# ggirelli/kman

Hardware: NVIDIA B200
Metric: k-mers/sec (extract+sort+count, k=31) (higher is better)
Workload: dtype u64

## Files before the change

### kman_b200/csrc/common.cuh

```cuda
#pragma once
#include <cuda_runtime.h>
#include <stdint.h>
#include <stdio.h>
#include <string.h>

#include <type_traits>

#include "../../include/kmg.h"

namespace kmg {

void set_error(const char* fmt, ...);
void bump_launches(int n = 1);

#define KMG_CUDA(call)                                                                          \
    do {                                                                                        \
        cudaError_t e__ = (call);                                                               \
        if (e__ != cudaSuccess) {                                                               \
            kmg::set_error("%s:%d: %s -> %s", __FILE__, __LINE__, #call, cudaGetErrorString(e__)); \
            return KMG_ERR_CUDA;                                                                \
        }                                                                                       \
    } while (0)

#define KMG_REQUIRE(cond, code, ...)    \
// ... 29 lines not shown
static inline PassPlan make_plan(int begin_bit, int end_bit) {
    PassPlan plan;
    memset(&plan, 0, sizeof(plan));
    const int bits = end_bit - begin_bit;
    const int np = (bits + SORT_RADIX_BITS - 1) / SORT_RADIX_BITS;
    plan.num_passes = np;
    for (int i = 0; i < np; ++i) {
        plan.shift[i] = begin_bit + i * SORT_RADIX_BITS;
        plan.bits[i] = i + 1 < np ? SORT_RADIX_BITS : bits - i * SORT_RADIX_BITS;
    }
    return plan;
}

struct CountOut {
    uint32_t* counts;
    unsigned long long* n_out;
    bool done;
};
struct PrePartitioned {
    int pb;
    const unsigned long long* top;
    const unsigned long long* bucket_starts = nullptr;
    bool in_alt = false;
};
size_t top_hist_workspace_bytes();
int extract_top_hist(const uint8_t* d_bases, uint64_t n_bases, uint64_t win_begin, uint64_t win_end, int k, int rc,
                     const uint8_t* d_lut256, uint64_t* d_counts, unsigned long long* d_top, unsigned long long* d_plan,
                     void* d_ws, size_t ws_bytes, cudaStream_t st);
constexpr size_t P16_ZEROED_WORDS = 65536 + 3 * 256 + 4;
static inline unsigned long long* p16_top(unsigned long long* zeroed) { return zeroed + 65536; }
static inline unsigned long long* p16_plan(unsigned long long* zeroed) { return zeroed + 65536 + 3 * 256; }
struct Prefix16Out {
    unsigned long long* zeroed;
    unsigned long long* region_starts;
    unsigned long long* starts;
    unsigned long long* cursors;
    uint32_t* rows;
};
size_t prefix16_rows_bytes();
int extract_prefix16_hist(const uint8_t* d_bases, uint64_t n_bases, uint64_t win_begin, uint64_t win_end, int k, int rc,
                          const uint8_t* d_lut256, const Prefix16Out& o, cudaStream_t st);
int region_partition(const void* d_keys_in, void* d_keys_out, const void* d_vals_in, void* d_vals_out, uint64_t n,
                     int key_bytes, int val_bytes, const unsigned long long* d_region_counts, unsigned long long* d_cursors,
                     int digit_shift, cudaStream_t st);
int extract_digit_scatter(const uint8_t* d_bases, uint64_t n_bases, uint64_t win_begin, uint64_t win_end, int k, int rc,
                          const uint8_t* d_lut256, void* d_keys_out, int key_bytes, void* d_vals_out, int val_bytes,
                          uint64_t pos_offset, unsigned long long* d_cursors, int digit_shift, cudaStream_t st);
bool hybrid_sort_applies(uint64_t n, int key_bytes, int val_bytes, int end_bit, bool pairs_ok);
int hybrid_choose_pb(uint64_t n, unsigned long long max_top_byte_count, int key_bytes, int val_bytes);
int sort_count_core(void* d_keys, void* d_keys_alt, uint64_t n, int key_bytes, int end_bit, const uint64_t* d_hist_in,
                    uint32_t* d_counts_out, uint64_t* d_n_out, int* h_selector_out, void* d_ws, size_t ws_bytes, void* stream,
                    const PrePartitioned* pre);
int sort_uniq_core(void* d_keys, void* d_keys_alt, void* d_vals, void* d_vals_alt, uint64_t n, int key_bytes, int val_bytes,
                   int end_bit, const uint64_t* d_hist_in, uint64_t* d_n_out, int* h_selector_out, void* d_ws,
                   size_t ws_bytes, void* stream, const PrePartitioned* pre);
void exclusive_scan_256(const unsigned long long* d_hist_row, unsigned long long* d_out, cudaStream_t st);
extern thread_local int64_t g_stat_last_n_out, g_stat_last_err;
void timing_begin(cudaStream_t st);
void timing_end(cudaStream_t st, int kind);

struct __align__(16) u128 {
    uint64_t lo, hi;
};

__host__ __device__ __forceinline__ bool operator==(const u128& a, const u128& b) { return a.lo == b.lo && a.hi == b.hi; }
__host__ __device__ __forceinline__ bool operator!=(const u128& a, const u128& b) { return !(a == b); }
__host__ __device__ __forceinline__ bool operator<(const u128& a, const u128& b) {
    return a.hi < b.hi || (a.hi == b.hi && a.lo < b.lo);
}

struct __align__(16) u256 {
    u128 lo, hi;
// ... 152 lines not shown
__device__ __forceinline__ void mbar_expect_tx(uint64_t* bar, uint32_t bytes) {
    asm volatile("mbarrier.arrive.expect_tx.shared::cta.b64 _, [%0], %1;" ::"r"(smem_u32(bar)), "r"(bytes) : "memory");
}
__device__ __forceinline__ void mbar_wait(uint64_t* bar, uint32_t parity) {
    asm volatile(
        "{\n"
        ".reg .pred p;\n"
        "WAIT_LOOP:\n"
        "mbarrier.try_wait.parity.shared::cta.b64 p, [%0], %1;\n"
        "@p bra WAIT_DONE;\n"
        "bra WAIT_LOOP;\n"
        "WAIT_DONE:\n"
        "}\n" ::"r"(smem_u32(bar)),
        "r"(parity)
        : "memory");
}
__device__ __forceinline__ void tma_load_1d(void* smem_dst, const void* gmem_src, uint32_t bytes, uint64_t* bar) {
    asm volatile("cp.async.bulk.shared::cluster.global.mbarrier::complete_tx::bytes [%0], [%1], %2, [%3];" ::"r"(
                     smem_u32(smem_dst)),
                 "l"(gmem_src), "r"(bytes), "r"(smem_u32(bar))
                 : "memory");
}

__device__ __forceinline__ void tma_prefetch_l2(const void* gmem_src, uint32_t bytes) {
    asm volatile("cp.async.bulk.prefetch.L2.global [%0], %1;" ::"l"(gmem_src), "r"(bytes) : "memory");
}

__device__ __forceinline__ uint32_t lane_id() { return threadIdx.x & 31; }
__device__ __forceinline__ uint32_t lanemask_lt() {
    uint32_t m;
    asm("mov.u32 %0, %%lanemask_lt;" : "=r"(m));
    return m;
}

template <typename T>
__device__ __forceinline__ T warp_incl_scan(T v) {
#pragma unroll
    for (int o = 1; o < 32; o <<= 1) {
        T t = __shfl_up_sync(0xffffffffu, v, o);
        if (lane_id() >= (uint32_t)o) v += t;
    }
    return v;
}

template <int BLOCK, typename T>
__device__ __forceinline__ T block_excl_scan(T v, T* smem, T& total) {
// ... 18 lines not shown
```

### kman_b200/csrc/extract.cu

```cuda
#include "extract_tile.cuh"

namespace kmg {

constexpr int EX_BLOCK_DEFAULT = 256;

struct ExtractParams {
    const uint8_t* bases;
    uint64_t n_bases;
    uint64_t win_begin, win_end;
    uint64_t first_tile;
    int k;
    const uint8_t* lut;
    const uint8_t* comp16;
    void* keys_out;
    void* vals_out;
    uint64_t pos_offset;
    unsigned long long* counts;
    uint64_t* tile_state;
    uint32_t* ticket;
    uint32_t* err;
    unsigned long long* hs;
    int n_off;
    int hist_off[2 * MAX_PASSES];
    unsigned long long* cursors;
// ... 13 lines not shown
__device__ __forceinline__ uint32_t mer4_at(uint64_t X0, uint64_t X1, uint64_t X2, int e) {
    const int w = e >> 5, off = 2 * (e & 31);
    const uint64_t a = w == 0 ? X0 : (w == 1 ? X1 : X2);
    const uint64_t b = w == 0 ? X1 : (w == 1 ? X2 : 0ull);
    const uint64_t v = off == 0 ? a : ((a << off) | (b >> (64 - off)));
    return (uint32_t)(v >> 56);
}
__device__ __forceinline__ bool plain4_at(uint64_t B0, uint64_t B1, int e) {
    uint64_t v;
    if (e == 0) v = B0;
    else if (e < 64) v = (B0 << e) | (B1 >> (64 - e));
    else v = B1 << (e - 64);
    return (v >> 60) == 0;
}

template <int BLOCK>
struct DigitRuns {
    uint32_t* s_cnt;
    uint32_t* s_off;
    unsigned long long* s_gb;
    uint32_t* s_scan;

    __device__ __forceinline__ uint32_t rank(uint32_t d) const { return d | (atomicAdd(&s_cnt[d], 1u) << 8); }
    __device__ __forceinline__ uint32_t reserve(unsigned long long* cursors) const {
        const int t = threadIdx.x;
        const uint32_t c = t < 256 ? s_cnt[t] : 0u;
        unsigned long long g = 0;
        if (c) g = atomicAdd(&cursors[t], (unsigned long long)c);
        uint32_t n_tile;
        const uint32_t off = block_excl_scan<BLOCK, uint32_t>(c, s_scan, n_tile);
        if (t < 256) {
            s_off[t] = off;
            s_gb[t] = g - off;
        }
        __syncthreads();
        return n_tile;
    }
    __device__ __forceinline__ uint32_t slot(uint32_t wh) const { return s_off[wh & 255u] + (wh >> 8); }
    template <bool PAY, typename KeyT, typename ValT, typename DigitOf>
    __device__ __forceinline__ void write_runs(const KeyT* s_keys, const ValT* s_vals, uint32_t n_tile, DigitOf digit_of,
                                               KeyT* keys_out, ValT* vals_out) const {
        for (uint32_t i = threadIdx.x; i < n_tile; i += BLOCK) {
            const KeyT key = s_keys[i];
            const unsigned long long at = s_gb[digit_of(key)] + i;
            keys_out[at] = key;
            if constexpr (PAY) vals_out[at] = s_vals[i];
        }
    }
};

template <typename KeyT, int PPT, bool RC, int VAL_BYTES, bool HIST, int MODE, int EX_BLOCK, bool FILTER = false>
// ... 112 lines not shown
        }
    }
    if constexpr (MODE == 1) {
        __syncthreads();
        if (t == 0) {
            if (total) atomicAdd(&p.counts[0], (unsigned long long)total * OUT_PER_WIN);
            if (s_wide) atomicAdd(&p.counts[1], (unsigned long long)s_wide);
        }
        return;
    }

    if constexpr (MODE == 2) {
        const int dsh = p.digit_shift;
        const DigitRuns<EX_BLOCK> runs{s_cnt, s_off, s_gb, s_scan};
        uint32_t wh[PPT * OUT_PER_WIN];
#pragma unroll
        for (int j = 0; j < PPT; ++j) {
            if (!(vf & (1u << j))) continue;
            const KeyT key = build_key<KeyT>(X0, X1, X2, joff + j, k);
            wh[j * OUT_PER_WIN] = runs.rank(key_digit(key, dsh, 255u));
            if constexpr (RC) wh[j * 2 + 1] = runs.rank(key_digit(rc_key(key, k), dsh, 255u));
        }
        __syncthreads();
        const uint32_t n_tile = runs.reserve(p.cursors);
#pragma unroll
        for (int j = 0; j < PPT; ++j) {
            if (!(vf & (1u << j))) continue;
            const KeyT key = build_key<KeyT>(X0, X1, X2, joff + j, k);
            const uint64_t pos = tile_pos + (uint64_t)t * PPT + j + p.pos_offset;
            const uint32_t i0 = runs.slot(wh[j * OUT_PER_WIN]);
            s_keys[i0] = key;
            if constexpr (VAL_BYTES != 0) s_vals[i0] = make_val<ValT>(pos, 0);
            if constexpr (RC) {
                const uint32_t i1 = runs.slot(wh[j * 2 + 1]);
                s_keys[i1] = rc_key(key, k);
                if constexpr (VAL_BYTES != 0) s_vals[i1] = make_val<ValT>(pos, 1);
            }
        }
        __syncthreads();
        runs.template write_runs<VAL_BYTES != 0>(s_keys, s_vals, n_tile, [dsh](const KeyT& key) { return key_digit(key, dsh, 255u); },
                                                 reinterpret_cast<KeyT*>(p.keys_out), reinterpret_cast<ValT*>(p.vals_out));
        return;
    }

    uint32_t r = excl;
#pragma unroll
    for (int j = 0; j < PPT; ++j) {
// ... 407 lines not shown
    if (t < 256) {
        s_lut[t] = p.lut[t];
        s_b3[t] = 0;
    }
    if (t < 2) s_n[t] = 0;
    const int k = p.k;
    uint32_t n_valid = 0, n_wide = 0;
    for (uint32_t tile = blockIdx.x; tile < p.n_tiles; tile += gridDim.x) {
        __syncthreads();
        const uint64_t tile_pos = (p.first_tile + tile) * P16_TILE;
        encode_tile_words<P16_BLOCK, WORDS>(p.bases, p.n_bases, t, tile_pos, s_lut, s_codes, s_bad, s_inv);
        __syncthreads();
        const auto [X0, X1, X2, B0, B1, I0, I1] = load_tile_words(s_codes, s_bad, s_inv, t);
        uint32_t in_range_mask, nwide;
        bool span_clean;
        const uint32_t vf = narrow_window_flags<P16_PPT>(tile_pos + (uint64_t)t * P16_PPT, p.win_begin, p.win_end, k, 0, B0, B1,
                                                         I0, I1, in_range_mask, span_clean, nwide);
        n_valid += __popc(vf);
        n_wide += nwide;
#pragma unroll
        for (int j = 0; j < P16_PPT; ++j) {
            if (!(vf & (1u << j))) continue;
            count16(s_h, p.spill, mer8_at(X0, X1, X2, j));
            atomicAdd(&s_b3[mer4_at(X0, X1, X2, j + 8)], 1u);
            if constexpr (RC) {
                count16(s_h, p.spill, rc8(mer8_at(X0, X1, X2, j + k - 8)));
                atomicAdd(&s_b3[rc4(mer4_at(X0, X1, X2, j + k - 12))], 1u);
            }
        }
    }
#pragma unroll
    for (int o = 16; o > 0; o >>= 1) {
        n_valid += __shfl_xor_sync(0xffffffffu, n_valid, o);
        n_wide += __shfl_xor_sync(0xffffffffu, n_wide, o);
    }
    if ((t & 31) == 0) {
        if (n_valid) atomicAdd(&s_n[0], (unsigned long long)n_valid);
        if (n_wide) atomicAdd(&s_n[1], (unsigned long long)n_wide);
    }
    __syncthreads();
    uint4* row = reinterpret_cast<uint4*>(p.rows + (size_t)blockIdx.x * P16_WORDS);
    for (uint32_t i = t; i < P16_WORDS / 4; i += P16_BLOCK) row[i] = reinterpret_cast<const uint4*>(s_h)[i];
    if (t < 256 && s_b3[t]) atomicAdd(&p.byte3[t], (unsigned long long)s_b3[t]);
    if (t < 2 && s_n[t]) atomicAdd(&p.counts[t], s_n[t]);
}

__global__ void __launch_bounds__(256) prefix16_reduce_kernel(const uint32_t* __restrict__ rows, int n_rows,
                                                              const unsigned long long* __restrict__ spill,
                                                              unsigned long long* __restrict__ top,
                                                              unsigned long long* __restrict__ starts) {
    __shared__ unsigned long long s_scan[256 / 32 + 1];
    const uint32_t r = blockIdx.x, t = threadIdx.x, b = r * 256 + t;
    const uint32_t* w = rows + (b >> 1);
    const int sh = (int)(b & 1u) << 4;
    uint32_t acc = 0;
#pragma unroll 8
    for (int c = 0; c < n_rows; ++c) acc += (w[(size_t)c * P16_WORDS] >> sh) & 0xFFFFu;
    const unsigned long long v = spill[b] + acc;
    unsigned long long tot;
    const unsigned long long ex = block_excl_scan<256, unsigned long long>(v, s_scan, tot);
    starts[b] = ex;
    if (t == 0) top[2 * 256 + r] = tot;
    if (v) atomicAdd(&top[256 + t], v);
}

__global__ void __launch_bounds__(256) prefix16_starts_kernel(const unsigned long long* __restrict__ top,
                                                              unsigned long long* __restrict__ plan,
                                                              unsigned long long* __restrict__ region_starts,
                                                              unsigned long long* __restrict__ starts,
                                                              unsigned long long* __restrict__ cursors) {
    __shared__ unsigned long long s_scan[256 / 32 + 1], s_max[8], s_base;
    const uint32_t r = blockIdx.x, t = threadIdx.x, b = r * 256 + t;
    const unsigned long long c = top[2 * 256 + t];
    unsigned long long total;
    const unsigned long long ex = block_excl_scan<256, unsigned long long>(c, s_scan, total);
    if (t == r) s_base = ex;
    __syncthreads();
    const unsigned long long s = starts[b] + s_base;
    starts[b] = s;
    cursors[b] = s;
    if (t == 0) region_starts[r] = s_base;
    if (r == 0) {
        unsigned long long mx = c;
#pragma unroll
        for (int o = 16; o > 0; o >>= 1) mx = max(mx, __shfl_xor_sync(0xffffffffu, mx, o));
        if ((t & 31) == 0) s_max[t >> 5] = mx;
        __syncthreads();
        if (t == 0) {
            for (int i = 1; i < 8; ++i) mx = max(mx, s_max[i]);
            plan[0] = total;
            plan[1] = mx;
            starts[65536] = total;
        }
    }
}

constexpr int RP_BLOCK = 512;
template <typename KeyT, int VB>
constexpr int rp_ipt() { return sizeof(KeyT) == 8 ? (VB == 0 ? 12 : 8) : (VB == 8 ? 6 : 8); }

struct RegionPartParams {
    const void* keys_in;
    void* keys_out;
    const void* vals_in;
    void* vals_out;
    const unsigned long long* counts;
    unsigned long long* cursors;
    int digit_shift;
};

template <typename KeyT, int VB>
__global__ void __launch_bounds__(RP_BLOCK, 2) region_partition_kernel(const RegionPartParams p) {
    constexpr int IPT = rp_ipt<KeyT, VB>();
    constexpr uint32_t TILE = RP_BLOCK * IPT;
    using ValT = typename std::conditional<VB == 4, uint32_t, uint64_t>::type;
    extern __shared__ __align__(16) unsigned char smem_raw[];
    KeyT* s_keys = reinterpret_cast<KeyT*>(smem_raw);
    ValT* s_vals = reinterpret_cast<ValT*>(smem_raw + sizeof(KeyT) * TILE);
    __shared__ uint32_t s_cnt[256], s_off[256];
    __shared__ unsigned long long s_gb[256];
    __shared__ uint32_t s_scan[RP_BLOCK / 32 + 1];
    __shared__ unsigned long long s_scan64[RP_BLOCK / 32 + 1];
    __shared__ uint32_t s_region;
    __shared__ unsigned long long s_lo, s_hi;

    const int t = threadIdx.x;
    const unsigned long long c = t < 256 ? p.counts[t] : 0ull;
    const uint32_t nt = (uint32_t)((c + TILE - 1) / TILE);
    uint32_t tiles_all;
    unsigned long long keys_all;
    const uint32_t t0 = block_excl_scan<RP_BLOCK, uint32_t>(nt, s_scan, tiles_all);
    const unsigned long long k0 = block_excl_scan<RP_BLOCK, unsigned long long>(c, s_scan64, keys_all);
    if (blockIdx.x >= tiles_all) return;
    if (t < 256) s_cnt[t] = 0;
    if (blockIdx.x - t0 < nt) {
        s_region = t;
        s_lo = k0 + (unsigned long long)(blockIdx.x - t0) * TILE;
        s_hi = k0 + c;
    }
    __syncthreads();
    const uint32_t r = s_region;
    const unsigned long long lo = s_lo;
    const uint32_t n_in = (uint32_t)min((unsigned long long)TILE, s_hi - lo);
    const KeyT* keys_in = reinterpret_cast<const KeyT*>(p.keys_in) + lo;
    const ValT* vals_in = reinterpret_cast<const ValT*>(p.vals_in) + lo;
    const int dsh = p.digit_shift;
    const DigitRuns<RP_BLOCK> runs{s_cnt, s_off, s_gb, s_scan};
    KeyT key[IPT];
    ValT val[VB ? IPT : 1];
    uint32_t wh[IPT];
#pragma unroll
    for (int q = 0; q < IPT; ++q) {
        const uint32_t i = q * RP_BLOCK + t;
        if (i < n_in) {
            key[q] = keys_in[i];
            if constexpr (VB != 0) val[q] = vals_in[i];
        }
    }
#pragma unroll
    for (int q = 0; q < IPT; ++q)
        if (q * RP_BLOCK + t < n_in) wh[q] = runs.rank(key_digit(key[q], dsh, 255u));
    __syncthreads();
    const uint32_t n_tile = runs.reserve(p.cursors + (size_t)r * 256);
#pragma unroll
    for (int q = 0; q < IPT; ++q) {
        if (q * RP_BLOCK + t < n_in) {
            const uint32_t i = runs.slot(wh[q]);
            s_keys[i] = key[q];
            if constexpr (VB != 0) s_vals[i] = val[q];
        }
    }
    __syncthreads();
    runs.template write_runs<VB != 0>(s_keys, s_vals, n_tile, [dsh](const KeyT& k_) { return key_digit(k_, dsh, 255u); },
                                      reinterpret_cast<KeyT*>(p.keys_out), reinterpret_cast<ValT*>(p.vals_out));
}

template <typename KeyT, int VB>
static int launch_region_partition(const RegionPartParams& p, uint64_t n, cudaStream_t st) {
    constexpr uint64_t TILE = (uint64_t)RP_BLOCK * rp_ipt<KeyT, VB>();
    const uint64_t grid = (n + TILE - 1) / TILE + 256;
    KMG_REQUIRE(grid < (1ull << 31), KMG_ERR_RANGE, "too many tiles");
    const size_t smem = TILE * (sizeof(KeyT) + VB);
    auto kern = region_partition_kernel<KeyT, VB>;
    KMG_CUDA(cudaFuncSetAttribute(kern, cudaFuncAttributeMaxDynamicSharedMemorySize, (int)smem));
    kern<<<(uint32_t)grid, RP_BLOCK, smem, st>>>(p);
    KMG_LAUNCH_CHECK();
    return KMG_OK;
}

template <bool RC, int LIMBS, int FILTER = 0>
static int dispatch_wide(const ExtractParams& p, uint32_t n_tiles, int vb, cudaStream_t st) {
    if (vb == 0) extract_wide_kernel<RC, 0, LIMBS, FILTER><<<n_tiles, EXW_BLOCK, 0, st>>>(p);
    else if (vb == 4) extract_wide_kernel<RC, 4, LIMBS, FILTER><<<n_tiles, EXW_BLOCK, 0, st>>>(p);
    else extract_wide_kernel<RC, 8, LIMBS, FILTER><<<n_tiles, EXW_BLOCK, 0, st>>>(p);
    KMG_LAUNCH_CHECK();
    return KMG_OK;
}
template <int FILTER>
static int dispatch_wide_any(const ExtractParams& p, uint32_t n_tiles, int k, int rc, int vb, cudaStream_t st) {
    if (k <= 32) return rc ? dispatch_wide<true, 2, FILTER>(p, n_tiles, vb, st) : dispatch_wide<false, 2, FILTER>(p, n_tiles, vb, st);
    return rc ? dispatch_wide<true, 4, FILTER>(p, n_tiles, vb, st) : dispatch_wide<false, 4, FILTER>(p, n_tiles, vb, st);
}

static void fill_common(ExtractParams& p, const uint8_t* d_bases, uint64_t n_bases, uint64_t win_begin, uint64_t win_end,
                        uint64_t tile, int k, const uint8_t* d_lut256) {
// ... 308 lines not shown
```

### kman_b200/csrc/pipeline.cu

```cuda
#include <algorithm>

#include "common.cuh"

extern "C" size_t kmg_rle_workspace_bytes(uint64_t n);

namespace kmg {

namespace {
struct PipeWs {
    unsigned long long* zeroed;
    unsigned long long* top;
    unsigned long long* plan;
    unsigned long long* cursors;
    unsigned long long* starts;
    unsigned long long* cursors16;
    uint32_t* rows;
    uint64_t* hist16;
    uint64_t* n_out;
    void* ex_ws;
    size_t ex_ws_bytes;
    void* sort_ws;
    size_t sort_ws_bytes;
    size_t total;
};
// ... 77 lines not shown
    if (fused) {
        timing_begin(st);
        const Prefix16Out p16{w.zeroed, w.cursors, w.starts, w.cursors16, w.rows};
        rcode = extract_prefix16_hist(d_bases, n_bases, win_begin, win_end, k, rc, d_lut256, p16, st);
        timing_end(st, 2);
        if (rcode != KMG_OK) return rcode;
        unsigned long long h_plan[4] = {0, 0, 0, 0};
        KMG_CUDA(cudaMemcpyAsync(h_plan, w.plan, sizeof(h_plan), cudaMemcpyDeviceToHost, st));
        KMG_CUDA(cudaStreamSynchronize(st));
        n = h_plan[0];
        h_result[1] = n;
        h_result[2] = h_plan[3];
        KMG_REQUIRE(h_plan[2] * (rc ? 2 : 1) == n, KMG_ERR_STATE,
                    "prefix histogram (%llu keys) disagrees with the window count (%llu)", h_plan[0],
                    h_plan[2] * (rc ? 2 : 1));
        if (n == 0) return KMG_OK;
        fused = hybrid_sort_applies(n, kb, val_bytes, 2 * k, true);
        if (fused) {
            PrePartitioned pre;
            pre.pb = hybrid_choose_pb(n, h_plan[1], kb, val_bytes);
            pre.top = w.top;
            const bool msd = pre.pb == 16;
            if (!msd) exclusive_scan_256(w.top, w.cursors, st);
            timing_begin(st);
            rcode = extract_digit_scatter(d_bases, n_bases, win_begin, win_end, k, rc, d_lut256, d_keys, kb, d_vals, val_bytes,
                                          pos_offset, w.cursors, msd ? 2 * k - 8 : 2 * k - 24, st);
            timing_end(st, 3);
            if (rcode != KMG_OK) return rcode;
            if (msd) {
                timing_begin(st);
                rcode = region_partition(d_keys, d_keys_alt, d_vals, d_vals_alt, n, kb, val_bytes, w.top + 2 * 256, w.cursors16,
                                         2 * k - 16, st);
                timing_end(st, 0);
                if (rcode != KMG_OK) return rcode;
                pre.bucket_starts = w.starts;
                pre.in_alt = true;
            }
            if (mode == 0)
                rcode = sort_count_core(d_keys, d_keys_alt, n, kb, 2 * k, nullptr, d_counts_out, w.n_out, &sel, w.sort_ws,
                                        w.sort_ws_bytes, st, &pre);
            else
                rcode = sort_uniq_core(d_keys, d_keys_alt, d_vals, d_vals_alt, n, kb, val_bytes, 2 * k, nullptr, w.n_out, &sel,
                                       w.sort_ws, w.sort_ws_bytes, st, &pre);
            if (rcode != KMG_OK) return rcode;
        }
    }
// ... 99 lines not shown
```

### kman_b200/csrc/radix_sort.cu

```cuda
#include <cmath>
#include <type_traits>

#include "common.cuh"

namespace kmg {

struct ShiftDigit {
    int shift;
    uint32_t mask;
    template <typename KeyT>
    __device__ __forceinline__ uint32_t operator()(const KeyT& k) const {
        return key_digit(k, shift, mask);
    }
};
struct RangeDigit {
    int shift;
    uint32_t n_parts;
    template <typename KeyT>
    __device__ __forceinline__ uint32_t operator()(const KeyT& k) const {
        return (key_digit(k, shift, 0xFFFFu) * n_parts) >> 16;
    }
};

template <typename KeyT, int RADIX_BITS>
// ... 515 lines not shown
    uint32_t ticket, err;
    unsigned long long irregular, big_runs;
    uint32_t ls_ticket, pad5;
    unsigned long long over_tiles, over_keys, n_out;
};
static_assert(sizeof(HybridHeaderView) == 56, "layout of the header words");

static int hybrid_tile_cap(int key_bytes, int val_bytes) {
    return key_bytes == 16 ? (val_bytes ? ls_cap<u128, true>() : ls_cap<u128, false>())
                           : (val_bytes ? ls_cap<uint64_t, true>() : ls_cap<uint64_t, false>());
}
static bool hybrid_pb16_ok(uint64_t n, unsigned long long max_top_byte_count, int key_bytes, int val_bytes) {
    const unsigned long long fullest = max_top_byte_count / 256;
    if (fullest <= (unsigned long long)(key_bytes == 16 ? 800 : (val_bytes ? 2500 : 3400))) return true;
    if (key_bytes == 16) return false;
    const double avg = (double)n / 65536.0;
    return (double)fullest <= 1.04 * avg && avg + 6.0 * std::sqrt(avg) <= (double)hybrid_tile_cap(key_bytes, val_bytes) - 64.0;
}
int hybrid_choose_pb(uint64_t n, unsigned long long max_top_byte_count, int key_bytes, int val_bytes) {
    if (g_hybrid_pb == 16 || g_hybrid_pb == 24) return g_hybrid_pb;
    return hybrid_pb16_ok(n, max_top_byte_count, key_bytes, val_bytes) ? 16 : 24;
}

static int sort_impl(void* d_keys, void* d_keys_alt, void* d_vals, void* d_vals_alt, uint64_t n, int key_bytes,
                     int val_bytes, int begin_bit, int end_bit, const uint64_t* d_hist_in, int* h_selector_out,
                     void* d_ws, size_t ws_bytes, cudaStream_t st, bool hybrid, bool allow_hybrid,
                     CountOut* co = nullptr, const PrePartitioned* pre = nullptr) {
    SortWs w = carve_sort_ws(d_ws, n, key_bytes, hybrid, val_bytes);
    KMG_REQUIRE(ws_bytes >= w.total, KMG_ERR_WS, "sort workspace too small: %zu < %zu", ws_bytes, w.total);
    hybrid = hybrid && allow_hybrid;
    KMG_REQUIRE(!pre || hybrid, KMG_ERR_ARG, "pre-partitioned keys need the hybrid finish");
    const bool prefix_done = pre && pre->bucket_starts;
    KMG_REQUIRE(!prefix_done || pre->pb == 16, KMG_ERR_ARG, "bucket starts come with the 16-bit prefix");

    PassPlan plan = make_plan(begin_bit, end_bit);
    int np = plan.num_passes;
    const uint64_t n_parts = (n + PART_MAX - 1) / PART_MAX;

    KMG_CUDA(cudaMemsetAsync(d_ws, 0, w.zero_bytes, st));

    int dev = 0, sms = 148;
    cudaGetDevice(&dev);
    cudaDeviceGetAttribute(&sms, cudaDevAttrMultiProcessorCount, dev);

    const unsigned long long* hist = w.hist;
    int pb = 0;
    if (hybrid) {
        memset(&plan, 0, sizeof(plan));
        plan.num_passes = 3;
        for (int i = 0; i < 3; ++i) {
            plan.shift[i] = end_bit - 24 + 8 * i;
            plan.bits[i] = 8;
        }
        if (pre) {
            if (!prefix_done)
                KMG_CUDA(cudaMemcpyAsync(w.hist, pre->top, (size_t)3 * SORT_RADIX * sizeof(uint64_t), cudaMemcpyDeviceToDevice, st));
        } else if (d_hist_in && key_bytes == 8 && (end_bit & 1) == 0) {
            KMG_CUDA(cudaMemcpyAsync(w.hist, d_hist_in + (size_t)13 * SORT_RADIX, (size_t)3 * SORT_RADIX * sizeof(uint64_t),
                                     cudaMemcpyDeviceToDevice, st));
        } else {
            const int grid = (int)std::min<uint64_t>((n + 511) / 512, (uint64_t)sms * 4);
            if (key_bytes == 8)
// ... 70 lines not shown
                    KMG_CUDA(cudaMemsetAsync(w.lookback, 0, (char*)d_ws + w.zero_bytes - (char*)w.lookback, st));
                p.tag = 1u << 30;
            } else {
                p.tag = (launch % 3u + 1u) << 30;
            }
            if (g_ev_used >= MAX_TIMED) timing_collect();
            timing_begin(st);
            int rcode = dispatch_onesweep(hybrid && pass == 0, key_bytes, val_bytes, p, op, st);
            timing_end(st, 0);
            if (rcode != KMG_OK) return rcode;
            ++launch;
        }
        std::swap(kin, kout);
        std::swap(vin, vout);
        ++g_stat_sort_passes;
    }
    if (!hybrid) {
        *h_selector_out = np & 1;
        return KMG_OK;
    }

    const bool wide_key = key_bytes == 16;
    const bool pairs = val_bytes != 0;
    const int cap = wide_key ? (pairs ? ls_cap<u128, true>() : ls_cap<u128, false>())
                             : (pairs ? ls_cap<uint64_t, true>() : ls_cap<uint64_t, false>());
    HybridParams hp;
    memset(&hp, 0, sizeof(hp));
    hp.keys_in = kin;
    hp.keys_out = kout;
    hp.vals_in = vin;
    hp.vals_out = vout;
    hp.n = n;
    const double avg = (double)n / (double)(1ull << pb);
    auto tile_width = [&](double want) {
        if (avg > cap / 2.4) return (uint32_t)std::max<double>(LS_T_MIN, std::min<double>(cap - 256, avg - 6.0 * std::sqrt(avg) - 8.0));
        double target = std::min<double>(want, cap - std::max(256.0, 1.35 * avg));
        target = std::max<double>(target, LS_T_MIN);
        if (avg < 64) return (uint32_t)target;
        const int kbk = std::max(1, (int)(target / avg));
        return (uint32_t)std::min<double>(cap - 256, std::max<double>(LS_T_MIN, std::ceil(kbk * avg)));
    };
    hp.bounds = w.hyb_bounds;
    hp.flag = w.hyb_flag;
    hp.off = w.hyb_off;
    hp.key_bits = end_bit;
    hp.pb = pb;
    HybridHeaderView* hv = reinterpret_cast<HybridHeaderView*>(w.hdr);
    hp.irregular = &hv->irregular;
    hp.over = &hv->over_tiles;
    hp.n_out_copy = &hv->n_out;
    hp.tile_state = w.hyb_state;
    hp.ticket = &hv->ls_ticket;
    hp.err = &w.hdr->err;
    const double avg_bucket = (double)n / (double)(1ull << pb);
    const bool few_bucket_tiles =
        avg_bucket > cap / 2.4 ||
        (avg_bucket >= 64 && std::min<double>(g_local_tile, cap - std::max(256.0, 1.35 * avg_bucket)) < 2.0 * avg_bucket);
    const bool fine = !few_bucket_tiles;
    const size_t smem = fine ? (wide_key ? (pairs ? lsf_smem_bytes<u128, true>() : lsf_smem_bytes<u128, false>())
                                         : (pairs ? lsf_smem_bytes<uint64_t, true>() : lsf_smem_bytes<uint64_t, false>()))
                             : (wide_key ? (pairs ? ls_smem_bytes<u128, true>() : ls_smem_bytes<u128, false>())
                                         : (pairs ? ls_smem_bytes<uint64_t, true>() : ls_smem_bytes<uint64_t, false>()));
    const int sel_in = kin == (char*)d_keys ? 0 : 1;
    const int sel_done = sel_in ^ 1;
    const bool want_fused = co != nullptr && g_count_fused;

    auto launch_bounds = [&](uint32_t T) -> int {
        hp.tile_t = T;
        hp.n_tiles = (uint32_t)((n + T - 1) / T);
        if (prefix_done) bounds_from_starts_kernel<<<(hp.n_tiles + 1 + 255) / 256, 256, 0, st>>>(hp, pre->bucket_starts, 1u << pb);
        else if (wide_key) tile_bounds_kernel<u128><<<(hp.n_tiles + 1 + 7) / 8, 256, 0, st>>>(hp);
        else tile_bounds_kernel<uint64_t><<<(hp.n_tiles + 1 + 7) / 8, 256, 0, st>>>(hp);
        KMG_LAUNCH_CHECK();
        KMG_CUDA(cudaMemsetAsync(hp.over, 0, 2 * sizeof(unsigned long long), st));
        oversize_tiles_kernel<<<(hp.n_tiles + 255) / 256, 256, 0, st>>>(hp, (uint32_t)cap, hp.over);
        KMG_LAUNCH_CHECK();
        return KMG_OK;
    };
    auto launch_local = [&](bool fused) -> int {
        hp.counts_out = fused ? co->counts : nullptr;
        hp.n_out = fused ? co->n_out : nullptr;
        if (g_ev_used >= MAX_TIMED) timing_collect();
        timing_begin(st);
#define KMG_LS_LAUNCH(K, E, V)                                                                                   \
    do {                                                                                                         \
        auto kern = fine ? local_sort_fine_kernel<K, E, V> : local_sort_kernel<K, E, V>;                         \
        KMG_CUDA(cudaFuncSetAttribute(kern, cudaFuncAttributeMaxDynamicSharedMemorySize, (int)smem));            \
                             \
        kern<<<fine ? std::min<uint32_t>(hp.n_tiles, 2u * (uint32_t)sms) : hp.n_tiles, LS_BLOCK, smem, st>>>(hp); \
    } while (0)
        if (fused && pairs && wide_key) {
            if (val_bytes == 4) KMG_LS_LAUNCH(u128, 2, 4);
            else KMG_LS_LAUNCH(u128, 2, 8);
        } else if (fused && pairs) {
// ... 7 lines not shown
            else KMG_LS_LAUNCH(u128, 0, 8);
        } else if (pairs) {
            if (val_bytes == 4) KMG_LS_LAUNCH(uint64_t, 0, 4);
            else KMG_LS_LAUNCH(uint64_t, 0, 8);
        } else {
            if (wide_key) KMG_LS_LAUNCH(u128, 0, 0);
            else KMG_LS_LAUNCH(uint64_t, 0, 0);
        }
#undef KMG_LS_LAUNCH
        timing_end(st, 1);
        KMG_LAUNCH_CHECK();
        return KMG_OK;
    };
    HybridHeaderView hh;
    auto read_header = [&]() -> int {
        KMG_CUDA(cudaMemcpyAsync(&hh, w.hdr, sizeof(hh), cudaMemcpyDeviceToHost, st));
        KMG_CUDA(cudaStreamSynchronize(st));
        g_stat_hybrid_irregular = (int64_t)hh.irregular;
        g_stat_hybrid_big_runs = (int64_t)hh.big_runs;
        g_stat_last_err = (int64_t)hh.err;
        return KMG_OK;
    };

    int rcode = launch_bounds(tile_width(g_local_tile));
    if (rcode != KMG_OK) return rcode;
    rcode = launch_local(want_fused);
    if (rcode != KMG_OK) return rcode;
    rcode = read_header();
    if (rcode != KMG_OK) return rcode;
    g_stat_hybrid_path = 1;
    if (hh.irregular == 0 && (!want_fused || hh.over_tiles == 0)) {
        if (want_fused) {
            co->done = true;
            g_stat_last_n_out = (int64_t)hh.n_out;
        }
        *h_selector_out = sel_done;
        return KMG_OK;
    }
    if (want_fused || hh.over_keys > n / 32) {
        const uint32_t cand[3] = {tile_width(g_local_tile), tile_width(cap / 2), tile_width(cap / 4)};
        if (hh.over_keys > n / 32) {
            for (int c = 1; c < 3; ++c) {
                if (cand[c] >= cand[c - 1]) continue;
                rcode = launch_bounds(cand[c]);
                if (rcode != KMG_OK) return rcode;
                rcode = read_header();
                if (rcode != KMG_OK) return rcode;
// ... 271 lines not shown
```

Measured before the change: 46.84 billion.

## Overlap hybrid bounds on side stream, persistent TMA region partition, signed byte3 hist

Computes the hybrid-sort tile bounds early on a side stream, overlapped with extract/scatter, and joins through an event before local sort. Turns region_partition into a persistent kernel that double-buffers TMA bulk loads of the next tile and writes out the previous tile's runs while reserving cursors for the current one, with smaller items-per-thread. Replaces the per-k-mer byte3 shared-memory histogram atomics with edge-difference signed updates, and folds the top histogram accumulation into the scan kernel. Adds cross-stream dependency and mbarrier/proxy-fence complexity, with more risk of ordering or correctness bugs.

```diff
diff --git a/kman_b200/csrc/common.cuh b/kman_b200/csrc/common.cuh
--- a/kman_b200/csrc/common.cuh
+++ b/kman_b200/csrc/common.cuh
@@ -75,6 +75,7 @@
     const unsigned long long* top;
     const unsigned long long* bucket_starts = nullptr;
     bool in_alt = false;
+    cudaEvent_t bounds_ready = nullptr;
 };
 size_t top_hist_workspace_bytes();
 int extract_top_hist(const uint8_t* d_bases, uint64_t n_bases, uint64_t win_begin, uint64_t win_end, int k, int rc,
@@ -101,6 +102,8 @@
                           uint64_t pos_offset, unsigned long long* d_cursors, int digit_shift, cudaStream_t st);
 bool hybrid_sort_applies(uint64_t n, int key_bytes, int val_bytes, int end_bit, bool pairs_ok);
 int hybrid_choose_pb(uint64_t n, unsigned long long max_top_byte_count, int key_bytes, int val_bytes);
+int hybrid_bounds_early(uint64_t n, int key_bytes, int val_bytes, const unsigned long long* bucket_starts, void* d_ws,
+                        size_t ws_bytes, cudaStream_t st, cudaEvent_t* ready);
 int sort_count_core(void* d_keys, void* d_keys_alt, uint64_t n, int key_bytes, int end_bit, const uint64_t* d_hist_in,
                     uint32_t* d_counts_out, uint64_t* d_n_out, int* h_selector_out, void* d_ws, size_t ws_bytes, void* stream,
                     const PrePartitioned* pre);
@@ -299,6 +302,8 @@
                  : "memory");
 }
 
+__device__ __forceinline__ void fence_proxy_async_shared() { asm volatile("fence.proxy.async.shared::cta;" ::: "memory"); }
+
 __device__ __forceinline__ void tma_prefetch_l2(const void* gmem_src, uint32_t bytes) {
     asm volatile("cp.async.bulk.prefetch.L2.global [%0], %1;" ::"l"(gmem_src), "r"(bytes) : "memory");
 }
diff --git a/kman_b200/csrc/extract.cu b/kman_b200/csrc/extract.cu
--- a/kman_b200/csrc/extract.cu
+++ b/kman_b200/csrc/extract.cu
@@ -59,11 +59,13 @@
     uint32_t* s_scan;
 
     __device__ __forceinline__ uint32_t rank(uint32_t d) const { return d | (atomicAdd(&s_cnt[d], 1u) << 8); }
-    __device__ __forceinline__ uint32_t reserve(unsigned long long* cursors) const {
+    template <typename Meanwhile>
+    __device__ __forceinline__ uint32_t reserve(unsigned long long* cursors, Meanwhile meanwhile) const {
         const int t = threadIdx.x;
         const uint32_t c = t < 256 ? s_cnt[t] : 0u;
         unsigned long long g = 0;
         if (c) g = atomicAdd(&cursors[t], (unsigned long long)c);
+        meanwhile();
         uint32_t n_tile;
         const uint32_t off = block_excl_scan<BLOCK, uint32_t>(c, s_scan, n_tile);
         if (t < 256) {
@@ -222,7 +224,7 @@
             if constexpr (RC) wh[j * 2 + 1] = runs.rank(key_digit(rc_key(key, k), dsh, 255u));
         }
         __syncthreads();
-        const uint32_t n_tile = runs.reserve(p.cursors);
+        const uint32_t n_tile = runs.reserve(p.cursors, [] {});
 #pragma unroll
         for (int j = 0; j < PPT; ++j) {
             if (!(vf & (1u << j))) continue;
@@ -676,11 +678,22 @@
         for (int j = 0; j < P16_PPT; ++j) {
             if (!(vf & (1u << j))) continue;
             count16(s_h, p.spill, mer8_at(X0, X1, X2, j));
-            atomicAdd(&s_b3[mer4_at(X0, X1, X2, j + 8)], 1u);
-            if constexpr (RC) {
-                count16(s_h, p.spill, rc8(mer8_at(X0, X1, X2, j + k - 8)));
-                atomicAdd(&s_b3[rc4(mer4_at(X0, X1, X2, j + k - 12))], 1u);
-            }
+            if constexpr (RC) count16(s_h, p.spill, rc8(mer8_at(X0, X1, X2, j + k - 8)));
+        }
+        uint32_t in8, nwide8;
+        bool clean8;
+        const uint32_t vf8 = narrow_window_flags<P16_PPT>(tile_pos + (uint64_t)t * P16_PPT + 8, p.win_begin, p.win_end, k, 8,
+                                                          B0, B1, I0, I1, in8, clean8, nwide8);
+        for (uint32_t edge = vf ^ vf8; edge; edge &= edge - 1u) {
+            const int j = __ffs(edge) - 1;
+            const uint32_t sgn = (vf >> j) & 1u ? 1u : ~0u;
+            atomicAdd(&s_b3[mer4_at(X0, X1, X2, j + 8)], sgn);
+            if constexpr (RC) atomicAdd(&s_b3[rc4(mer4_at(X0, X1, X2, j + k - 4))], 0u - sgn);
+        }
+        for (uint32_t head = tile == 0 && t == 0 ? vf & 0xFFu : 0u; head; head &= head - 1u) {
+            const int j = __ffs(head) - 1;
+            atomicAdd(&s_b3[mer4_at(X0, X1, X2, j)], ~0u);
+            if constexpr (RC) atomicAdd(&s_b3[rc4(mer4_at(X0, X1, X2, j + k - 12))], 1u);
         }
     }
 #pragma unroll
@@ -695,7 +708,7 @@
     __syncthreads();
     uint4* row = reinterpret_cast<uint4*>(p.rows + (size_t)blockIdx.x * P16_WORDS);
     for (uint32_t i = t; i < P16_WORDS / 4; i += P16_BLOCK) row[i] = reinterpret_cast<const uint4*>(s_h)[i];
-    if (t < 256 && s_b3[t]) atomicAdd(&p.byte3[t], (unsigned long long)s_b3[t]);
+    if (t < 256 && s_b3[t]) atomicAdd(&p.byte3[t], (unsigned long long)(long long)(int)s_b3[t]);
     if (t < 2 && s_n[t]) atomicAdd(&p.counts[t], s_n[t]);
 }
 
@@ -714,7 +727,10 @@
     unsigned long long tot;
     const unsigned long long ex = block_excl_scan<256, unsigned long long>(v, s_scan, tot);
     starts[b] = ex;
-    if (t == 0) top[2 * 256 + r] = tot;
+    if (t == 0) {
+        top[2 * 256 + r] = tot;
+        top[r] += tot;
+    }
     if (v) atomicAdd(&top[256 + t], v);
 }
 
@@ -750,8 +766,15 @@
 }
 
 constexpr int RP_BLOCK = 512;
+constexpr int RP_CTAS_PER_SM = 2;
 template <typename KeyT, int VB>
-constexpr int rp_ipt() { return sizeof(KeyT) == 8 ? (VB == 0 ? 12 : 8) : (VB == 8 ? 6 : 8); }
+constexpr int rp_ipt() {
+    return sizeof(KeyT) == 8 ? (VB == 0 ? 12 : 6) : (VB == 0 ? 6 : 4);
+}
+template <typename KeyT, int VB>
+constexpr size_t rp_smem() {
+    return (size_t)RP_BLOCK * rp_ipt<KeyT, VB>() * 2 * (sizeof(KeyT) + VB) + 16 * (VB ? 2 : 1);
+}
 
 struct RegionPartParams {
     const void* keys_in;
@@ -763,20 +786,42 @@
     int digit_shift;
 };
 
+template <int B>
+struct RpSpan {
+    uint64_t x0, a0, b0;
+    __device__ __forceinline__ RpSpan(const void* g, unsigned long long lo, uint32_t n)
+        : x0((uint64_t)g + lo * B), a0((x0 + 15) & ~15ull), b0((x0 + (uint64_t)n * B) & ~15ull) {}
+    __device__ __forceinline__ uint32_t bytes() const { return b0 > a0 ? (uint32_t)(b0 - a0) : 0u; }
+    __device__ __forceinline__ uint32_t a() const { return bytes() ? (uint32_t)((a0 - x0) / B) : 0u; }
+    __device__ __forceinline__ uint32_t b() const { return bytes() ? (uint32_t)((b0 - x0) / B) : 0u; }
+    __device__ __forceinline__ uint32_t shift() const { return (uint32_t)(x0 & 15); }
+    __device__ __forceinline__ void load(unsigned char* s_buf, uint64_t* bar) const {
+        constexpr uint32_t CHUNK = 16384;
+        const uint32_t n = bytes();
+        for (uint32_t o = 0; o < n; o += CHUNK)
+            tma_load_1d(s_buf + (a0 - (x0 & ~15ull)) + o, reinterpret_cast<const void*>(a0 + o), min(CHUNK, n - o), bar);
+    }
+};
+
 template <typename KeyT, int VB>
-__global__ void __launch_bounds__(RP_BLOCK, 2) region_partition_kernel(const RegionPartParams p) {
+__global__ void __launch_bounds__(RP_BLOCK, RP_CTAS_PER_SM) region_partition_kernel(const RegionPartParams p) {
     constexpr int IPT = rp_ipt<KeyT, VB>();
     constexpr uint32_t TILE = RP_BLOCK * IPT;
+    constexpr int KB = sizeof(KeyT);
     using ValT = typename std::conditional<VB == 4, uint32_t, uint64_t>::type;
     extern __shared__ __align__(16) unsigned char smem_raw[];
-    KeyT* s_keys = reinterpret_cast<KeyT*>(smem_raw);
-    ValT* s_vals = reinterpret_cast<ValT*>(smem_raw + sizeof(KeyT) * TILE);
-    __shared__ uint32_t s_cnt[256], s_off[256];
-    __shared__ unsigned long long s_gb[256];
+    unsigned char* in_keys = smem_raw;
+    unsigned char* in_vals = smem_raw + TILE * KB + 16;
+    KeyT* s_keys = reinterpret_cast<KeyT*>(smem_raw + (TILE * KB + 16) + (VB ? TILE * VB + 16 : 0));
+    ValT* s_vals = reinterpret_cast<ValT*>(reinterpret_cast<unsigned char*>(s_keys) + TILE * KB);
+    __shared__ uint32_t s_cnt[256], s_off[256], s_t0[256];
+    __shared__ unsigned long long s_gb[2][256];
+    __shared__ unsigned long long s_k0[257];
     __shared__ uint32_t s_scan[RP_BLOCK / 32 + 1];
     __shared__ unsigned long long s_scan64[RP_BLOCK / 32 + 1];
-    __shared__ uint32_t s_region;
-    __shared__ unsigned long long s_lo, s_hi;
+    __shared__ unsigned long long s_lo[2];
+    __shared__ uint32_t s_n[2], s_r[2];
+    __shared__ __align__(8) uint64_t s_bar;
 
     const int t = threadIdx.x;
     const unsigned long long c = t < 256 ? p.counts[t] : 0ull;
@@ -786,55 +831,110 @@
     const uint32_t t0 = block_excl_scan<RP_BLOCK, uint32_t>(nt, s_scan, tiles_all);
     const unsigned long long k0 = block_excl_scan<RP_BLOCK, unsigned long long>(c, s_scan64, keys_all);
     if (blockIdx.x >= tiles_all) return;
-    if (t < 256) s_cnt[t] = 0;
-    if (blockIdx.x - t0 < nt) {
-        s_region = t;
-        s_lo = k0 + (unsigned long long)(blockIdx.x - t0) * TILE;
-        s_hi = k0 + c;
-    }
-    __syncthreads();
-    const uint32_t r = s_region;
-    const unsigned long long lo = s_lo;
-    const uint32_t n_in = (uint32_t)min((unsigned long long)TILE, s_hi - lo);
-    const KeyT* keys_in = reinterpret_cast<const KeyT*>(p.keys_in) + lo;
-    const ValT* vals_in = reinterpret_cast<const ValT*>(p.vals_in) + lo;
+    if (t < 256) {
+        s_cnt[t] = 0;
+        s_t0[t] = t0;
+        s_k0[t] = k0;
+    }
+    if (t == 0) {
+        s_k0[256] = keys_all;
+        mbar_init(&s_bar, 1);
+    }
+    __syncthreads();
+    auto fetch = [&](uint32_t tile, uint32_t s) {
+        int a = 0, b = 256;
+        while (a < b) {
+            const int m = (a + b) >> 1;
+            if (s_t0[m] <= tile) a = m + 1;
+            else b = m;
+        }
+        const uint32_t r = (uint32_t)(a - 1);
+        const unsigned long long lo = s_k0[r] + (unsigned long long)(tile - s_t0[r]) * TILE;
+        const uint32_t n = (uint32_t)min((unsigned long long)TILE, s_k0[r + 1] - lo);
+        s_lo[s] = lo;
+        s_n[s] = n;
+        s_r[s] = r;
+        const RpSpan<KB> sk(p.keys_in, lo, n);
+        const RpSpan<VB ? VB : 4> sv(p.vals_in, lo, n);
+        fence_proxy_async_shared();
+        mbar_expect_tx(&s_bar, sk.bytes() + (VB ? sv.bytes() : 0u));
+        sk.load(in_keys, &s_bar);
+        if constexpr (VB != 0) sv.load(in_vals, &s_bar);
+    };
+    if (t == 0) fetch(blockIdx.x, 0);
+    __syncthreads();
+
     const int dsh = p.digit_shift;
-    const DigitRuns<RP_BLOCK> runs{s_cnt, s_off, s_gb, s_scan};
-    KeyT key[IPT];
-    ValT val[VB ? IPT : 1];
-    uint32_t wh[IPT];
-#pragma unroll
-    for (int q = 0; q < IPT; ++q) {
-        const uint32_t i = q * RP_BLOCK + t;
-        if (i < n_in) {
-            key[q] = keys_in[i];
-            if constexpr (VB != 0) val[q] = vals_in[i];
-        }
-    }
-#pragma unroll
-    for (int q = 0; q < IPT; ++q)
-        if (q * RP_BLOCK + t < n_in) wh[q] = runs.rank(key_digit(key[q], dsh, 255u));
-    __syncthreads();
-    const uint32_t n_tile = runs.reserve(p.cursors + (size_t)r * 256);
-#pragma unroll
-    for (int q = 0; q < IPT; ++q) {
-        if (q * RP_BLOCK + t < n_in) {
-            const uint32_t i = runs.slot(wh[q]);
-            s_keys[i] = key[q];
-            if constexpr (VB != 0) s_vals[i] = val[q];
-        }
-    }
-    __syncthreads();
-    runs.template write_runs<VB != 0>(s_keys, s_vals, n_tile, [dsh](const KeyT& k_) { return key_digit(k_, dsh, 255u); },
-                                      reinterpret_cast<KeyT*>(p.keys_out), reinterpret_cast<ValT*>(p.vals_out));
+    auto digit_of = [dsh](const KeyT& k_) { return key_digit(k_, dsh, 255u); };
+    KeyT* keys_out = reinterpret_cast<KeyT*>(p.keys_out);
+    ValT* vals_out = reinterpret_cast<ValT*>(p.vals_out);
+    uint32_t n_prev = 0, par = 0;
+    for (uint32_t tile = blockIdx.x; tile < tiles_all; tile += gridDim.x, par ^= 1u) {
+        const unsigned long long lo = s_lo[par];
+        const uint32_t n_in = s_n[par], r = s_r[par];
+        KeyT key[IPT];
+        ValT val[VB ? IPT : 1];
+        uint32_t wh[IPT];
+        mbar_wait(&s_bar, par);
+        {
+            const RpSpan<KB> sk(p.keys_in, lo, n_in);
+            const uint32_t a = sk.a(), b = sk.b();
+            const KeyT* sin = reinterpret_cast<const KeyT*>(in_keys + sk.shift());
+            const KeyT* gin = reinterpret_cast<const KeyT*>(p.keys_in) + lo;
+#pragma unroll
+            for (int q = 0; q < IPT; ++q) {
+                const uint32_t i = q * RP_BLOCK + t;
+                if (i < n_in) key[q] = i - a < b - a ? sin[i] : gin[i];
+            }
+        }
+        if constexpr (VB != 0) {
+            const RpSpan<VB> sv(p.vals_in, lo, n_in);
+            const uint32_t a = sv.a(), b = sv.b();
+            const ValT* sin = reinterpret_cast<const ValT*>(in_vals + sv.shift());
+            const ValT* gin = reinterpret_cast<const ValT*>(p.vals_in) + lo;
+#pragma unroll
+            for (int q = 0; q < IPT; ++q) {
+                const uint32_t i = q * RP_BLOCK + t;
+                if (i < n_in) val[q] = i - a < b - a ? sin[i] : gin[i];
+            }
+        }
+        __syncthreads();
+        if (t == 0 && tile + gridDim.x < tiles_all) fetch(tile + gridDim.x, par ^ 1u);
+        const DigitRuns<RP_BLOCK> runs{s_cnt, s_off, s_gb[par], s_scan};
+        const DigitRuns<RP_BLOCK> prev{s_cnt, s_off, s_gb[par ^ 1u], s_scan};
+#pragma unroll
+        for (int q = 0; q < IPT; ++q)
+            if (q * RP_BLOCK + t < n_in) wh[q] = runs.rank(digit_of(key[q]));
+        __syncthreads();
+        const uint32_t n_tile = runs.reserve(p.cursors + (size_t)r * 256, [&] {
+            prev.template write_runs<VB != 0>(s_keys, s_vals, n_prev, digit_of, keys_out, vals_out);
+        });
+        if (t < 256) s_cnt[t] = 0;
+#pragma unroll
+        for (int q = 0; q < IPT; ++q) {
+            if (q * RP_BLOCK + t < n_in) {
+                const uint32_t i = runs.slot(wh[q]);
+                s_keys[i] = key[q];
+                if constexpr (VB != 0) s_vals[i] = val[q];
+            }
+        }
+        n_prev = n_tile;
+    }
+    __syncthreads();
+    const DigitRuns<RP_BLOCK> last{s_cnt, s_off, s_gb[par ^ 1u], s_scan};
+    last.template write_runs<VB != 0>(s_keys, s_vals, n_prev, digit_of, keys_out, vals_out);
 }
 
 template <typename KeyT, int VB>
 static int launch_region_partition(const RegionPartParams& p, uint64_t n, cudaStream_t st) {
     constexpr uint64_t TILE = (uint64_t)RP_BLOCK * rp_ipt<KeyT, VB>();
-    const uint64_t grid = (n + TILE - 1) / TILE + 256;
-    KMG_REQUIRE(grid < (1ull << 31), KMG_ERR_RANGE, "too many tiles");
-    const size_t smem = TILE * (sizeof(KeyT) + VB);
+    const uint64_t tiles = (n + TILE - 1) / TILE + 256;
+    KMG_REQUIRE(tiles < (1ull << 31), KMG_ERR_RANGE, "too many tiles");
+    int dev = 0, sms = 148;
+    KMG_CUDA(cudaGetDevice(&dev));
+    KMG_CUDA(cudaDeviceGetAttribute(&sms, cudaDevAttrMultiProcessorCount, dev));
+    const uint64_t grid = std::min<uint64_t>(tiles, (uint64_t)sms * RP_CTAS_PER_SM);
+    constexpr size_t smem = rp_smem<KeyT, VB>();
     auto kern = region_partition_kernel<KeyT, VB>;
     KMG_CUDA(cudaFuncSetAttribute(kern, cudaFuncAttributeMaxDynamicSharedMemorySize, (int)smem));
     kern<<<(uint32_t)grid, RP_BLOCK, smem, st>>>(p);
diff --git a/kman_b200/csrc/pipeline.cu b/kman_b200/csrc/pipeline.cu
--- a/kman_b200/csrc/pipeline.cu
+++ b/kman_b200/csrc/pipeline.cu
@@ -123,6 +123,10 @@
             pre.top = w.top;
             const bool msd = pre.pb == 16;
             if (!msd) exclusive_scan_256(w.top, w.cursors, st);
+            if (msd) {
+                rcode = hybrid_bounds_early(n, kb, val_bytes, w.starts, w.sort_ws, w.sort_ws_bytes, st, &pre.bounds_ready);
+                if (rcode != KMG_OK) return rcode;
+            }
             timing_begin(st);
             rcode = extract_digit_scatter(d_bases, n_bases, win_begin, win_end, k, rc, d_lut256, d_keys, kb, d_vals, val_bytes,
                                           pos_offset, w.cursors, msd ? 2 * k - 8 : 2 * k - 24, st);
diff --git a/kman_b200/csrc/radix_sort.cu b/kman_b200/csrc/radix_sort.cu
--- a/kman_b200/csrc/radix_sort.cu
+++ b/kman_b200/csrc/radix_sort.cu
@@ -561,6 +561,70 @@
     return hybrid_pb16_ok(n, max_top_byte_count, key_bytes, val_bytes) ? 16 : 24;
 }
 
+static int hybrid_cap(int key_bytes, int val_bytes) {
+    return key_bytes == 16 ? (val_bytes ? ls_cap<u128, true>() : ls_cap<u128, false>())
+                           : (val_bytes ? ls_cap<uint64_t, true>() : ls_cap<uint64_t, false>());
+}
+
+static uint32_t hybrid_tile_width(uint64_t n, int pb, int cap, double want) {
+    const double avg = (double)n / (double)(1ull << pb);
+    if (avg > cap / 2.4) return (uint32_t)std::max<double>(LS_T_MIN, std::min<double>(cap - 256, avg - 6.0 * std::sqrt(avg) - 8.0));
+    double target = std::min<double>(want, cap - std::max(256.0, 1.35 * avg));
+    target = std::max<double>(target, LS_T_MIN);
+    if (avg < 64) return (uint32_t)target;
+    const int kbk = std::max(1, (int)(target / avg));
+    return (uint32_t)std::min<double>(cap - 256, std::max<double>(LS_T_MIN, std::ceil(kbk * avg)));
+}
+
+static void launch_bounds_from_starts(HybridParams& hp, uint32_t T, const unsigned long long* starts, int cap, cudaStream_t st) {
+    hp.tile_t = T;
+    hp.n_tiles = (uint32_t)((hp.n + T - 1) / T);
+    bounds_from_starts_kernel<<<(hp.n_tiles + 1 + 255) / 256, 256, 0, st>>>(hp, starts, 1u << 16);
+    oversize_tiles_kernel<<<(hp.n_tiles + 255) / 256, 256, 0, st>>>(hp, (uint32_t)cap, hp.over);
+}
+
+struct SideStream {
+    cudaStream_t s = nullptr;
+    cudaEvent_t fork = nullptr, join = nullptr;
+};
+static int side_stream(SideStream*& out) {
+    thread_local SideStream per_dev[64];
+    int dev = 0;
+    KMG_CUDA(cudaGetDevice(&dev));
+    KMG_REQUIRE(dev >= 0 && dev < 64, KMG_ERR_RANGE, "device %d", dev);
+    SideStream& x = per_dev[dev];
+    if (!x.s) {
+        KMG_CUDA(cudaStreamCreateWithFlags(&x.s, cudaStreamNonBlocking));
+        KMG_CUDA(cudaEventCreateWithFlags(&x.fork, cudaEventDisableTiming));
+        KMG_CUDA(cudaEventCreateWithFlags(&x.join, cudaEventDisableTiming));
+    }
+    out = &x;
+    return KMG_OK;
+}
+
+int hybrid_bounds_early(uint64_t n, int key_bytes, int val_bytes, const unsigned long long* bucket_starts, void* d_ws,
+                        size_t ws_bytes, cudaStream_t st, cudaEvent_t* ready) {
+    const SortWs w = carve_sort_ws(d_ws, n, key_bytes, true, val_bytes);
+    KMG_REQUIRE(ws_bytes >= w.total, KMG_ERR_WS, "sort workspace too small: %zu < %zu", ws_bytes, w.total);
+    SideStream* ss = nullptr;
+    const int rcode = side_stream(ss);
+    if (rcode != KMG_OK) return rcode;
+    KMG_CUDA(cudaMemsetAsync(d_ws, 0, w.zero_bytes, st));
+    KMG_CUDA(cudaEventRecord(ss->fork, st));
+    KMG_CUDA(cudaStreamWaitEvent(ss->s, ss->fork, 0));
+    HybridParams hp;
+    memset(&hp, 0, sizeof(hp));
+    hp.n = n;
+    hp.bounds = w.hyb_bounds;
+    hp.over = &reinterpret_cast<HybridHeaderView*>(w.hdr)->over_tiles;
+    const int cap = hybrid_cap(key_bytes, val_bytes);
+    launch_bounds_from_starts(hp, hybrid_tile_width(n, 16, cap, g_local_tile), bucket_starts, cap, ss->s);
+    KMG_LAUNCH_CHECK();
+    KMG_CUDA(cudaEventRecord(ss->join, ss->s));
+    *ready = ss->join;
+    return KMG_OK;
+}
+
 static int sort_impl(void* d_keys, void* d_keys_alt, void* d_vals, void* d_vals_alt, uint64_t n, int key_bytes,
                      int val_bytes, int begin_bit, int end_bit, const uint64_t* d_hist_in, int* h_selector_out,
                      void* d_ws, size_t ws_bytes, cudaStream_t st, bool hybrid, bool allow_hybrid,
@@ -576,7 +640,9 @@
     int np = plan.num_passes;
     const uint64_t n_parts = (n + PART_MAX - 1) / PART_MAX;
 
-    KMG_CUDA(cudaMemsetAsync(d_ws, 0, w.zero_bytes, st));
+    const bool bounds_early = prefix_done && pre->bounds_ready;
+
+    if (!bounds_early) KMG_CUDA(cudaMemsetAsync(d_ws, 0, w.zero_bytes, st));
 
     int dev = 0, sms = 148;
     cudaGetDevice(&dev);
@@ -693,8 +759,7 @@
 
     const bool wide_key = key_bytes == 16;
     const bool pairs = val_bytes != 0;
-    const int cap = wide_key ? (pairs ? ls_cap<u128, true>() : ls_cap<u128, false>())
-                             : (pairs ? ls_cap<uint64_t, true>() : ls_cap<uint64_t, false>());
+    const int cap = hybrid_cap(key_bytes, val_bytes);
     HybridParams hp;
     memset(&hp, 0, sizeof(hp));
     hp.keys_in = kin;
@@ -702,15 +767,7 @@
     hp.vals_in = vin;
     hp.vals_out = vout;
     hp.n = n;
-    const double avg = (double)n / (double)(1ull << pb);
-    auto tile_width = [&](double want) {
-        if (avg > cap / 2.4) return (uint32_t)std::max<double>(LS_T_MIN, std::min<double>(cap - 256, avg - 6.0 * std::sqrt(avg) - 8.0));
-        double target = std::min<double>(want, cap - std::max(256.0, 1.35 * avg));
-        target = std::max<double>(target, LS_T_MIN);
-        if (avg < 64) return (uint32_t)target;
-        const int kbk = std::max(1, (int)(target / avg));
-        return (uint32_t)std::min<double>(cap - 256, std::max<double>(LS_T_MIN, std::ceil(kbk * avg)));
-    };
+    auto tile_width = [&](double want) { return hybrid_tile_width(n, pb, cap, want); };
     hp.bounds = w.hyb_bounds;
     hp.flag = w.hyb_flag;
     hp.off = w.hyb_off;
@@ -739,8 +796,13 @@
     auto launch_bounds = [&](uint32_t T) -> int {
         hp.tile_t = T;
         hp.n_tiles = (uint32_t)((n + T - 1) / T);
-        if (prefix_done) bounds_from_starts_kernel<<<(hp.n_tiles + 1 + 255) / 256, 256, 0, st>>>(hp, pre->bucket_starts, 1u << pb);
-        else if (wide_key) tile_bounds_kernel<u128><<<(hp.n_tiles + 1 + 7) / 8, 256, 0, st>>>(hp);
+        if (prefix_done) {
+            KMG_CUDA(cudaMemsetAsync(hp.over, 0, 2 * sizeof(unsigned long long), st));
+            launch_bounds_from_starts(hp, T, pre->bucket_starts, cap, st);
+            KMG_LAUNCH_CHECK();
+            return KMG_OK;
+        }
+        if (wide_key) tile_bounds_kernel<u128><<<(hp.n_tiles + 1 + 7) / 8, 256, 0, st>>>(hp);
         else tile_bounds_kernel<uint64_t><<<(hp.n_tiles + 1 + 7) / 8, 256, 0, st>>>(hp);
         KMG_LAUNCH_CHECK();
         KMG_CUDA(cudaMemsetAsync(hp.over, 0, 2 * sizeof(unsigned long long), st));
@@ -794,7 +856,14 @@
         return KMG_OK;
     };
 
-    int rcode = launch_bounds(tile_width(g_local_tile));
+    int rcode = KMG_OK;
+    if (bounds_early) {
+        hp.tile_t = tile_width(g_local_tile);
+        hp.n_tiles = (uint32_t)((n + hp.tile_t - 1) / hp.tile_t);
+        KMG_CUDA(cudaStreamWaitEvent(st, pre->bounds_ready, 0));
+    } else {
+        rcode = launch_bounds(tile_width(g_local_tile));
+    }
     if (rcode != KMG_OK) return rcode;
     rcode = launch_local(want_fused);
     if (rcode != KMG_OK) return rcode;
```

Result: faster. 49.40 billion, median of 6 (+5.5%).
